# b0nes164/GPUSorting

Hardware: NVIDIA H100
Metric: OneSweep sort throughput, 2^30 uint32 keys per GPU, keys-only, uniform-random (higher is better)
Workload: dtype u32

## Files before the change

### gpusorting_b200/csrc/osb_kernels.cu

```cuda
#include <type_traits>

#include "osb_kernels.cuh"
#include "osb_common.cuh"

namespace osb {

template <typename... Ts> struct TypeList {};

template <typename... Ts, typename F>
static cudaError_t for_each_type(TypeList<Ts...>, F&& f)
{
    cudaError_t e = cudaSuccess;
    (void)(((e = f(Ts{})) == cudaSuccess) && ...);
    return e;
}

template <typename... Ts, typename M, typename F>
static cudaError_t find_type(TypeList<Ts...>, M&& match, F&& f)
{
    cudaError_t e = cudaErrorInvalidValue;
    (void)((match(Ts{}) && ((e = f(Ts{})), true)) || ...);
    return e;
}

template <typename... Keys, typename F>
static cudaError_t with_key_type(TypeList<Keys...> keys, int key_bytes, F&& f)
{
    return find_type(keys, [&](auto k) { return key_bytes == static_cast<int>(sizeof(k)); }, f);
}

template <typename F>
static cudaError_t with_rank_mode(int rank_mode, F&& f)
{
    return rank_mode == kRankBallot ? f(std::integral_constant<int, kRankBallot>{}) : f(std::integral_constant<int, kRankAtomic>{});
}

static unsigned capped_grid(uint64_t work, uint64_t per_cta, uint64_t cap)
{
    uint64_t want = (work + per_cta - 1) / per_cta;
    if (want < 1) want = 1;
    return static_cast<unsigned>(want < cap ? want : cap);
}

constexpr uint64_t kAllResident = ~0ull;
template <auto Kern, int THREADS, size_t SMEM, typename... Args>
static cudaError_t launch_resident(uint64_t max_ctas, int sm_count, cudaStream_t stream, Args... args)
{
    static const int per_sm = [] {
        int b = 0;
        return cudaOccupancyMaxActiveBlocksPerMultiprocessor(&b, Kern, THREADS, SMEM) == cudaSuccess ? b : 0;
    }();
    if (per_sm <= 0) return cudaErrorLaunchOutOfResources;
    const uint64_t ctas = static_cast<uint64_t>(per_sm) * sm_count;
    Kern<<<static_cast<unsigned>(max_ctas < ctas ? max_ctas : ctas), THREADS, SMEM, stream>>>(args...);
    return cudaGetLastError();
}

template <typename K>
static cudaError_t set_smem(K* kernel, size_t bytes)
{
    return cudaFuncSetAttribute(kernel, cudaFuncAttributeMaxDynamicSharedMemorySize, static_cast<int>(bytes));
}

template <typename Shape>
// ... 48 lines not shown
        v.x = enc2(v.x); v.y = enc2(v.y); v.z = enc2(v.z); v.w = enc2(v.w);
    } else {
        unsigned long long k0 = (static_cast<unsigned long long>(v.y) << 32) | v.x, k1 = (static_cast<unsigned long long>(v.w) << 32) | v.z;
        k0 = codec_encode<unsigned long long>(k0, c.a, c.b, c.d); k1 = codec_encode<unsigned long long>(k1, c.a, c.b, c.d);
        v.x = static_cast<uint32_t>(k0); v.y = static_cast<uint32_t>(k0 >> 32); v.z = static_cast<uint32_t>(k1); v.w = static_cast<uint32_t>(k1 >> 32);
    }
    return v;
}

template <typename KeyT, bool MASKED = false>
__device__ __forceinline__ void hist_count_vec(uint32_t* s_col, const uint4& v, int places = 0, uint32_t last_mask = 255u)
{
    hist_count_word<KeyT, MASKED>(s_col, v.x, 0, places, last_mask);
    hist_count_word<KeyT, MASKED>(s_col, v.y, 1, places, last_mask);
    hist_count_word<KeyT, MASKED>(s_col, v.z, 2, places, last_mask);
    hist_count_word<KeyT, MASKED>(s_col, v.w, 3, places, last_mask);
}

template <typename KeyT, bool MASKED = false>
__global__ void __launch_bounds__(kHistThreads, 1)
global_histogram_kernel(const KeyT* __restrict__ keys, uint64_t n, unsigned long long* __restrict__ ghist, KeyCodec codec,
                        int places = 0, uint32_t last_mask = 255u, const SortPlan* gate = nullptr)
{
    if (gate != nullptr && (gate->skip_mask & kPlanFusedKept)) return;
    constexpr int PLACES = sizeof(KeyT);
    constexpr int VEC = 16 / sizeof(KeyT);
    constexpr int COLS = HistGeom<KeyT>::COLS;
    constexpr int BINS = PLACES * kRadix;
    extern __shared__ __align__(16) uint32_t s_hist[];
    for (int i = threadIdx.x; i < BINS * COLS; i += kHistThreads) s_hist[i] = 0;
    __syncthreads();
    uint32_t* s_col = s_hist + (threadIdx.x & (COLS - 1));

    const uint64_t nvec = n / VEC;
    const uint4* __restrict__ vp = reinterpret_cast<const uint4*>(keys);
    const uint64_t stride = static_cast<uint64_t>(gridDim.x) * kHistThreads;
    uint64_t i = static_cast<uint64_t>(blockIdx.x) * kHistThreads + threadIdx.x;
    const bool enc = codec.flags & kCodecEncodeOnLoad;
    for (; i + 3 * stride < nvec; i += 4 * stride) {
        uint4 a = __ldcs(vp + i);
        uint4 b = __ldcs(vp + i + stride);
        uint4 c = __ldcs(vp + i + 2 * stride);
        uint4 d = __ldcs(vp + i + 3 * stride);
        if (enc) { a = hist_encode_vec<KeyT>(a, codec); b = hist_encode_vec<KeyT>(b, codec); c = hist_encode_vec<KeyT>(c, codec); d = hist_encode_vec<KeyT>(d, codec); }
        hist_count_vec<KeyT, MASKED>(s_col, a, places, last_mask);
        hist_count_vec<KeyT, MASKED>(s_col, b, places, last_mask);
// ... 18 lines not shown
            }
        }
    }
    __syncthreads();
    for (int bin = threadIdx.x; bin < BINS; bin += kHistThreads) {
        uint32_t sum = 0;
#pragma unroll 8
        for (int c = 0; c < COLS; ++c) sum += s_hist[bin * COLS + ((c + threadIdx.x) & (COLS - 1))];
        if (sum) atomicAdd(&ghist[bin], static_cast<unsigned long long>(sum));
    }
}

template <typename KeyT> constexpr size_t hist_smem_bytes() { return sizeof(KeyT) * kRadix * HistGeom<KeyT>::COLS * sizeof(uint32_t); }

using HistKeys = TypeList<uint16_t, uint32_t, uint64_t>;
using HistBitsKeys = TypeList<uint32_t, uint64_t>;

template <typename KeyT, bool MASKED>
static cudaError_t launch_histogram_vec(const void* keys, uint64_t n, unsigned long long* ghist, int sm_count, cudaStream_t stream,
                                        const KeyCodec& codec, int places = 0, uint32_t last_mask = 255u,
                                        const SortPlan* gate = nullptr)
{
    const unsigned grid = capped_grid(n / (16 / sizeof(KeyT)), kHistThreads, sm_count);
    global_histogram_kernel<KeyT, MASKED><<<grid, kHistThreads, hist_smem_bytes<KeyT>(), stream>>>(
        static_cast<const KeyT*>(keys), n, ghist, codec, places, last_mask, gate);
    return cudaGetLastError();
}

cudaError_t launch_global_histogram(const void* keys, uint64_t n, int key_bytes, unsigned long long* ghist,
                                    int sm_count, cudaStream_t stream, const KeyCodec* codec_in, const SortPlan* gate)
{
    const KeyCodec codec = codec_in ? *codec_in : KeyCodec();
    return with_key_type(HistKeys{}, key_bytes, [&](auto k) {
        return launch_histogram_vec<decltype(k), false>(keys, n, ghist, sm_count, stream, codec, 0, 255u, gate);
    });
}

__global__ void __launch_bounds__(512)
fused_fallback_zero_kernel(const SortPlan* __restrict__ plan, const uint32_t* __restrict__ ticket, uint32_t ctas, uint64_t tiles,
                           uint4* __restrict__ agg16, uint4* __restrict__ desc)
{
    if (plan->skip_mask & kPlanFusedKept) return;
    uint64_t reached = static_cast<uint64_t>(ctas) + *ticket;
    if (reached > tiles) reached = tiles;
    const uint64_t agg_vecs = (reached + 7) / 8 * 8 * kRadix * sizeof(uint16_t) / 16;
    const uint64_t desc_vecs = reached * kRadix * sizeof(uint64_t) / 16;
    const uint64_t stride = static_cast<uint64_t>(gridDim.x) * blockDim.x;
    for (uint64_t i = static_cast<uint64_t>(blockIdx.x) * blockDim.x + threadIdx.x; i < agg_vecs + desc_vecs; i += stride)
        (i < agg_vecs ? agg16[i] : desc[i - agg_vecs]) = make_uint4(0, 0, 0, 0);
}

cudaError_t launch_fused_fallback_zero(const SortPlan* plan, const uint32_t* ticket, uint32_t ctas, uint64_t tiles, uint16_t* agg16,
                                       uint64_t* desc, int sm_count, cudaStream_t stream)
{
    fused_fallback_zero_kernel<<<static_cast<unsigned>(sm_count) * 4, 512, 0, stream>>>(plan, ticket, ctas, tiles,
                                                                                         reinterpret_cast<uint4*>(agg16),
                                                                                         reinterpret_cast<uint4*>(desc));
    return cudaGetLastError();
}

template <typename KeyT>
__global__ void __launch_bounds__(kHistThreads, 1)
digit_histogram_kernel(const KeyT* __restrict__ keys, uint64_t n, uint32_t shift, unsigned long long* __restrict__ hist256)
{
    __shared__ uint32_t s_hist[kRadix * 32];
    for (int i = threadIdx.x; i < kRadix * 32; i += kHistThreads) s_hist[i] = 0;
    __syncthreads();
    uint32_t* s_col = s_hist + (threadIdx.x & 31);
    const uint64_t stride = static_cast<uint64_t>(gridDim.x) * kHistThreads;
    uint64_t i = static_cast<uint64_t>(blockIdx.x) * kHistThreads + threadIdx.x;
    for (; i + 3 * stride < n; i += 4 * stride) {
        const KeyT a = __ldcs(keys + i), b = __ldcs(keys + i + stride), c = __ldcs(keys + i + 2 * stride),
                   d = __ldcs(keys + i + 3 * stride);
        atomicAdd(&s_col[digit_of(a, shift) * 32], 1u);
        atomicAdd(&s_col[digit_of(b, shift) * 32], 1u);
        atomicAdd(&s_col[digit_of(c, shift) * 32], 1u);
        atomicAdd(&s_col[digit_of(d, shift) * 32], 1u);
    }
    for (; i < n; i += stride) atomicAdd(&s_col[digit_of(__ldcs(keys + i), shift) * 32], 1u);
    __syncthreads();
    for (int bin = threadIdx.x; bin < kRadix; bin += kHistThreads) {
// ... 3 lines not shown
        if (sum) atomicAdd(&hist256[bin], static_cast<unsigned long long>(sum));
    }
}

cudaError_t launch_digit_histogram(const void* keys, uint64_t n, int key_bytes, uint32_t shift,
                                   unsigned long long* hist256, int sm_count, cudaStream_t stream)
{
    const unsigned grid = capped_grid(n, kHistThreads * 4, static_cast<uint64_t>(sm_count) * 2);
    return with_key_type(TypeList<uint32_t, uint64_t>{}, key_bytes, [&](auto k) {
        using KeyT = decltype(k);
        digit_histogram_kernel<KeyT><<<grid, kHistThreads, 0, stream>>>(static_cast<const KeyT*>(keys), n, shift, hist256);
        return cudaGetLastError();
    });
}

enum ScanMode : int { kScanClassic = 0, kScanFused = 1, kScanFallback = 2 };

__global__ void __launch_bounds__(kRadix)
scan_kernel(const unsigned long long* __restrict__ ghist, unsigned long long* __restrict__ gbase, int places,
            SortPlan* plan, unsigned long long n, int allow_skip, int allow_hot, int mode, const uint32_t* fused_abort,
            unsigned long long region)
{
    __shared__ unsigned long long s_warp[kRadix / 32];
    if (mode == kScanFallback && (plan->skip_mask & kPlanFusedKept)) return;
    const int d = threadIdx.x, lane = d & 31, warp = d >> 5;
    uint32_t skip_mask = 0;
    const int overfull = mode == kScanFused ? __syncthreads_or(ghist[d] > region || *fused_abort != 0) : 0;
    for (int p = 0; p < places; ++p) {
        const unsigned long long c = ghist[p * kRadix + d];
        unsigned long long incl = c;
#pragma unroll
        for (int o = 1; o < 32; o <<= 1) {
            const unsigned long long t = __shfl_up_sync(0xffffffffu, incl, o);
            if (lane >= o) incl += t;
        }
        if (lane == 31) s_warp[warp] = incl;
        const int single_bin = __syncthreads_or(plan != nullptr && allow_skip && c == n);
        const int hot_bin = __syncthreads_or(plan != nullptr && allow_hot && n >= (1ull << 22) && c * 8ull >= n);
        unsigned long long pre = 0;
        for (int w = 0; w < warp; ++w) pre += s_warp[w];
        gbase[p * kRadix + d] = pre + incl - c;
        if (single_bin) skip_mask |= 1u << p;
        else if (hot_bin) skip_mask |= 1u << (kPlanHotShift + p);
        __syncthreads();
    }
    if (plan != nullptr && d == 0) {
        SortPlan pl;
        pl.skip_mask = skip_mask;
        const uint32_t run = ~skip_mask & ((places >= 32 ? 0u : (1u << places)) - 1u);
        pl.executed = __popc(run);
        pl.first_exec = run ? static_cast<uint32_t>(__ffs(run) - 1) : 0xffffffffu;
        pl.last_exec = run ? static_cast<uint32_t>(31 - __clz(run)) : 0xffffffffu;
        if (mode == kScanFused && !overfull && (run & 1u) && !((skip_mask >> kPlanHotShift) & 1u) && (run & ~1u))
            pl.skip_mask |= kPlanFusedKept;
        *plan = pl;
    }
}

cudaError_t launch_scan(const unsigned long long* ghist, unsigned long long* gbase, int places, cudaStream_t stream,
                        SortPlan* plan, uint64_t n, bool allow_skip, bool allow_hot)
{
    scan_kernel<<<1, kRadix, 0, stream>>>(ghist, gbase, places, plan, n, allow_skip ? 1 : 0, allow_hot ? 1 : 0, kScanClassic,
                                          nullptr, 0ull);
    return cudaGetLastError();
}

cudaError_t launch_scan_fused(const unsigned long long* ghist, unsigned long long* gbase, int places, cudaStream_t stream,
                              SortPlan* plan, uint64_t n, bool allow_skip, bool allow_hot, bool fallback, const uint32_t* fused_abort,
                              uint64_t region)
{
    scan_kernel<<<1, kRadix, 0, stream>>>(ghist, gbase, places, plan, n, allow_skip ? 1 : 0, allow_hot ? 1 : 0,
                                          fallback ? kScanFallback : kScanFused, fused_abort, region);
    return cudaGetLastError();
}

template <typename KeyT>
__global__ void __launch_bounds__(kHistThreads, 1)
global_histogram_bits_kernel(const KeyT* __restrict__ keys, uint64_t n, unsigned long long* __restrict__ ghist, KeyCodec codec,
                             uint32_t begin_bit, int places, uint32_t last_mask)
{
    constexpr int COLS = HistGeom<KeyT>::COLS;
    extern __shared__ __align__(16) uint32_t s_hist[];
    const int bins = places * kRadix;
    for (int i = threadIdx.x; i < bins * COLS; i += kHistThreads) s_hist[i] = 0;
    __syncthreads();
    uint32_t* s_col = s_hist + (threadIdx.x & (COLS - 1));
    const bool enc = codec.flags & kCodecEncodeOnLoad;
    const KeyT ca = static_cast<KeyT>(codec.a), cb = static_cast<KeyT>(codec.b), cd = static_cast<KeyT>(codec.d);
    const uint64_t stride = static_cast<uint64_t>(gridDim.x) * kHistThreads;
    for (uint64_t i = static_cast<uint64_t>(blockIdx.x) * kHistThreads + threadIdx.x; i < n; i += stride) {
        KeyT k = __ldcs(keys + i);
        if (enc) k = codec_encode<KeyT>(k, ca, cb, cd);
        for (int p = 0; p < places; ++p) {
            const uint32_t dg = digit_of(k, begin_bit + 8u * p, p == places - 1 ? last_mask : 255u);
            atomicAdd(&s_col[(p * kRadix + dg) * COLS], 1u);
        }
    }
    __syncthreads();
    for (int bin = threadIdx.x; bin < bins; bin += kHistThreads) {
        uint32_t sum = 0;
#pragma unroll 8
        for (int c = 0; c < COLS; ++c) sum += s_hist[bin * COLS + ((c + threadIdx.x) & (COLS - 1))];
        if (sum) atomicAdd(&ghist[bin], static_cast<unsigned long long>(sum));
    }
}

cudaError_t launch_global_histogram_bits(const void* keys, uint64_t n, int key_bytes, unsigned long long* ghist, int sm_count,
                                         cudaStream_t stream, const KeyCodec* codec_in, uint32_t begin_bit, int places,
                                         uint32_t last_bits)
{
    const KeyCodec codec = codec_in ? *codec_in : KeyCodec();
    const uint32_t last_mask = (1u << last_bits) - 1u;
    return with_key_type(HistBitsKeys{}, key_bytes, [&](auto k) {
        using KeyT = decltype(k);
        if (begin_bit == 0) return launch_histogram_vec<KeyT, true>(keys, n, ghist, sm_count, stream, codec, places, last_mask);
        global_histogram_bits_kernel<KeyT><<<capped_grid(n, kHistThreads * 4, sm_count), kHistThreads, hist_smem_bytes<KeyT>(), stream>>>(
            static_cast<const KeyT*>(keys), n, ghist, codec, begin_bit, places, last_mask);
        return cudaGetLastError();
    });
}

template <typename W>
__global__ void __launch_bounds__(512)
copy_back_kernel(const SortPlan* __restrict__ plan, const W* __restrict__ src, W* __restrict__ dst, uint64_t words,
                 const unsigned char* __restrict__ src_tail, unsigned char* __restrict__ dst_tail, uint32_t tail_bytes)
{
    if (!(plan->executed & 1u)) return;
    const uint64_t stride = static_cast<uint64_t>(gridDim.x) * blockDim.x;
    for (uint64_t i = static_cast<uint64_t>(blockIdx.x) * blockDim.x + threadIdx.x; i < words; i += stride) __stcs(dst + i, __ldcs(src + i));
    if (blockIdx.x == 0 && threadIdx.x < tail_bytes) dst_tail[threadIdx.x] = src_tail[threadIdx.x];
}

cudaError_t launch_copy_back(const SortPlan* plan, const void* alt_keys, void* keys, const uint32_t* alt_vals, uint32_t* vals,
                             uint64_t n, int key_bytes, int sm_count, cudaStream_t stream)
{
    auto launch = [&](auto word, const void* s, void* d, uint64_t bytes) {
        using W = decltype(word);
        const uint64_t words = bytes / sizeof(W);
        copy_back_kernel<W><<<capped_grid(words, 512, static_cast<uint64_t>(sm_count) * 4), 512, 0, stream>>>(plan, static_cast<const W*>(s), static_cast<W*>(d), words,
                                                      static_cast<const unsigned char*>(s) + words * sizeof(W),
                                                      static_cast<unsigned char*>(d) + words * sizeof(W),
                                                      static_cast<uint32_t>(bytes - words * sizeof(W)));
    };
    auto one = [&](const void* s, void* d, uint64_t bytes) {
        if (((reinterpret_cast<uintptr_t>(s) | reinterpret_cast<uintptr_t>(d)) & 15u) == 0) launch(uint4{}, s, d, bytes);
        else launch(uint32_t{}, s, d, bytes);
    };
    one(alt_keys, keys, n * key_bytes);
    if (vals) one(alt_vals, vals, n * sizeof(uint32_t));
    return cudaGetLastError();
}

template <typename KeyT>
__global__ void __launch_bounds__(512)
argsort_copy_back_kernel(const SortPlan* __restrict__ plan, const KeyT* __restrict__ keys_in, const KeyT* __restrict__ alt_keys,
                         KeyT* __restrict__ keys, const uint32_t* __restrict__ alt_idx, uint32_t* __restrict__ idx, uint64_t n)
{
    using KV = typename std::conditional<sizeof(KeyT) == 2, uint2, uint4>::type;
    constexpr int KV_PER_STEP = 4 * sizeof(KeyT) / sizeof(KV);
    static_assert(KV_PER_STEP * sizeof(KV) == 4 * sizeof(KeyT), "four keys per step");
    const uint32_t ex = plan->executed;
    if (ex != 0 && !(ex & 1u)) return;
    const KeyT* src = ex ? alt_keys : keys_in;
    const uint64_t vecs = n / 4, stride = static_cast<uint64_t>(gridDim.x) * blockDim.x;
    for (uint64_t i = static_cast<uint64_t>(blockIdx.x) * blockDim.x + threadIdx.x; i < vecs; i += stride) {
#pragma unroll
        for (int v = 0; v < KV_PER_STEP; ++v)
            __stcs(reinterpret_cast<KV*>(keys) + i * KV_PER_STEP + v, __ldcs(reinterpret_cast<const KV*>(src) + i * KV_PER_STEP + v));
        const uint32_t b = static_cast<uint32_t>(i * 4);
        __stcs(reinterpret_cast<uint4*>(idx) + i, ex ? __ldcs(reinterpret_cast<const uint4*>(alt_idx) + i) : make_uint4(b, b + 1, b + 2, b + 3));
    }
    if (blockIdx.x == 0 && threadIdx.x < (n & 3u)) {
        const uint64_t j = vecs * 4 + threadIdx.x;
        keys[j] = src[j];
        idx[j] = ex ? alt_idx[j] : static_cast<uint32_t>(j);
    }
}

cudaError_t launch_argsort_copy_back(const SortPlan* plan, const void* keys_in, const void* alt_keys, void* keys,
                                     const uint32_t* alt_idx, uint32_t* idx, uint64_t n, int key_bytes, int sm_count,
                                     cudaStream_t stream)
{
    const unsigned grid = capped_grid(n / 4, 512, static_cast<uint64_t>(sm_count) * 4);
    return with_key_type(TypeList<uint16_t, uint32_t, uint64_t>{}, key_bytes, [&](auto k) {
        using KeyT = decltype(k);
        argsort_copy_back_kernel<KeyT><<<grid, 512, 0, stream>>>(plan, static_cast<const KeyT*>(keys_in), static_cast<const KeyT*>(alt_keys),
                                                                 static_cast<KeyT*>(keys), alt_idx, idx, n);
        return cudaGetLastError();
    });
}


__device__ __forceinline__ uint32_t warp_match_digit(uint32_t d)
{
    uint32_t m = 0xffffffffu;
#pragma unroll
    for (int b = 0; b < kRadixLog; ++b) {
        const bool p = (d >> b) & 1u;
        const uint32_t bal = __ballot_sync(0xffffffffu, p);
        m &= p ? bal : ~bal;
    }
    return m;
}

template <int RANK_MODE>
__device__ __forceinline__ uint32_t warp_rank_and_count(uint32_t* wh, uint32_t d, uint32_t lt_mask)
{
    if constexpr (RANK_MODE == kRankAtomic) {
        (void)lt_mask;
        return atomicAdd(&wh[d], 1u);
    } else {
// ... 258 lines not shown
    for (uint32_t i = 0; i < tile_keys; ++i) {
        KeyT k = p[i];
        if (encode) k = codec_encode<KeyT>(k, ca, cb, cd);
        c += digit_of(k, shift, mask) == d;
    }
    st_relaxed_gpu_u16(dst, kAggReady | c);
    return c;
}

__device__ __forceinline__ uint64_t agg_index(uint64_t tile, uint32_t d) { return ((tile >> 3) * kRadix + d) * 8 + (tile & 7); }

__device__ __forceinline__ uint4 ld_relaxed_gpu_v4(const void* p)
{
    uint4 v;
    asm volatile("ld.relaxed.gpu.global.v4.u32 {%0, %1, %2, %3}, [%4];" : "=r"(v.x), "=r"(v.y), "=r"(v.z), "=r"(v.w) : "l"(p) : "memory");
    return v;
}
__device__ __forceinline__ uint32_t agg_elem(const uint4& v, int t)
{
    const uint32_t w = t < 2 ? v.x : t < 4 ? v.y : t < 6 ? v.z : v.w;
    return (t & 1) ? (w >> 16) : (w & 0xffffu);
}

template <int NBLK, typename KeyT, typename Hook = NoStallHook>
__device__ __forceinline__ unsigned long long
lookback_wide(uint16_t* agg16, const uint64_t* incl64, uint32_t tile, uint32_t d, uint32_t epoch, uint32_t spin_cap,
              const TileRereduce<KeyT>& rr, Hook hook = Hook())
{
    unsigned long long sum = 0;
    int64_t cur = static_cast<int64_t>(tile) - 1;
    uint32_t polls = 0;
    while (true) {
        if (cur < 0) return sum;
#if OSB_PHASE_PROBE
        if (d == 0) atomicAdd(&g_phase[9], 1ull);
#endif
        const int64_t b0 = cur >> 3;
        uint4 v[NBLK];
        uint64_t c[NBLK];
#pragma unroll
        for (int k = 0; k < NBLK; ++k) {
            const int64_t b = b0 - k;
            v[k] = b >= 0 ? ld_relaxed_gpu_v4(agg16 + (static_cast<uint64_t>(b) * kRadix + d) * 8)
                          : make_uint4(0x80008000u, 0x80008000u, 0x80008000u, 0x80008000u);
            c[k] = b > 0 ? ld_relaxed_gpu_u64(incl64 + (static_cast<uint64_t>(b) * 8 - 1) * kRadix + d) : 0ull;
        }
// ... 1 lines not shown
        int64_t next = (b0 - NBLK + 1) * 8 - 1;
        bool stalled = false;
        const int hi0 = static_cast<int>(cur & 7);
#pragma unroll
        for (int k = 0; k < NBLK; ++k) {
            const int64_t b = b0 - k;
            if (b < 0) return run;
#pragma unroll
            for (int t = 7; t >= 0; --t) {
                if (k == 0 && t > hi0) continue;
                const uint32_t a = agg_elem(v[k], t);
                if (!(a & kAggReady)) { next = b * 8 + t; stalled = true; break; }
                run += a & 0x7fffu;
            }
            if (stalled) break;
            if (b == 0) return run;
            if (desc_epoch(c[k]) == epoch && (c[k] & kFlagMask) == kFlagInclusive) return run + desc_value(c[k]);
        }
        sum = run;
        if (stalled) {
            if (hook(-1) == kHookAbort) return sum;
            polls = next == cur ? polls + 1 : 1;
            if (polls > spin_cap) {
                const uint64_t w = ld_relaxed_gpu_u64(incl64 + next * kRadix + d);
                if (desc_epoch(w) == epoch && (w & kFlagMask) == kFlagInclusive) return sum + desc_value(w);
                const long long h = hook(next);
                if (h >= 0)
                    sum += static_cast<unsigned long long>(h);
                else
                    sum += rereduce_tile<KeyT>(rr.in + static_cast<uint64_t>(next) * rr.tile_keys, rr.tile_keys, rr.shift, rr.mask,
                                               rr.encode ? 1u : 0u, rr.ca, rr.cb, rr.cd, agg16 + agg_index(next, d), d);
                --next;
                polls = 0;
            } else {
#if OSB_PHASE_PROBE
                if (d == 0) atomicAdd(&g_phase[10], 1ull);
#endif
                __nanosleep(40);
            }
        } else {
            polls = 0;
        }
        cur = next;
    }
}


constexpr uint32_t kNoHotDigit = 0xffffffffu;
// ... 87 lines not shown
                  (sizeof(KeyT) == 8 && sizeof(S::sorted) == sizeof(KeyT) * T && sizeof(S::sorted_val) == sizeof(uint32_t) * T),
                  "kv layout");
    uint2* const kv = reinterpret_cast<uint2*>(sm.sorted);
    auto put_slot = [&](uint32_t slot, KeyT k, uint32_t v) {
        if constexpr (KV_WORD) kv[slot] = make_uint2(static_cast<uint32_t>(k), v);
        else { sm.sorted[slot] = k; sm.sorted_val[slot] = v; }
    };
    auto get_slot = [&](uint32_t x, KeyT& k, uint32_t& v) {
        if constexpr (KV_WORD) { const uint2 e = kv[x]; k = static_cast<KeyT>(e.x); v = e.y; }
        else { k = sm.sorted[x]; v = sm.sorted_val[x]; }
    };

    const int tid = threadIdx.x, lane = tid & 31, warp = tid >> 5;
    const uint32_t lt = lanemask_lt();
    uint32_t* wh = sm.hist + warp * kRadix;
    const uint32_t shift = pp.shift, epoch = pp.epoch;
    const uint32_t dmask = (1u << pp.dbits) - 1u;
#if OSB_PHASE_PROBE
    long long t_prev = clock64();
#endif

    uint32_t my_bits = (codec.flags & (kCodecEncodeOnLoad | kCodecDecodeOnStore)) << 1;
    bool my_skip = false, my_hot = false;
    if (pp.plan != nullptr) {
        const uint4 raw = __ldg(reinterpret_cast<const uint4*>(pp.plan));
        SortPlan pl; pl.skip_mask = raw.x; pl.executed = raw.y; pl.first_exec = raw.z; pl.last_exec = raw.w;
        my_skip = (pl.skip_mask >> pp.place) & 1u;
        my_hot = (pl.skip_mask >> (kPlanHotShift + pp.place)) & 1u;
        my_bits = plan_src_is_alt(pl, pp.place) ? 1u : 0u;
        if (codec.flags & kCodecFromPlan)
            my_bits |= (pp.place == pl.first_exec ? kCodecEncodeOnLoad << 1 : 0u) | (pp.place == pl.last_exec ? kCodecDecodeOnStore << 1 : 0u);
        if constexpr (INDICES) my_bits |= pp.place == pl.first_exec ? kPlanBitsFirstIndices : 0u;
        if constexpr (S::kFusable) my_bits |= plan_reads_gapped(pl, pp.place) ? kPlanBitsGapped : 0u;
        if (pp.place == 0 && (pl.skip_mask & kPlanFusedKept)) my_skip = true;
    }
    if (my_skip) return;
    if (HOT != my_hot) return;
    const uint32_t num_tiles = static_cast<uint32_t>((n + T - 1) / T);

    using KeyReg = typename std::conditional<sizeof(KeyT) == 2 && !PAIRS, uint32_t, KeyT>::type;
    KeyReg key[K];
    uint32_t val[PAIRS ? K : 1];
    const uint32_t warp_off = warp * (32 * K) + lane;
    auto region_of = [&](uint64_t p) {
        uint32_t r = 0;
#pragma unroll 1
// ... 126 lines not shown

    auto chained_scan = [&]() {
        if (tid < kRadix) {
            TileRereduce<KeyT> rr;
            rr.in = (INDICES && (sm.plan_bits & kPlanBitsFirstIndices)) ? static_cast<const KeyT*>(pp.keys_in)
                    : (sm.plan_bits & 1u) ? buf1 : buf0;
            rr.tile_keys = T; rr.shift = shift; rr.mask = dmask;
            rr.encode = (sm.plan_bits >> 1) & kCodecEncodeOnLoad;
            rr.ca = static_cast<KeyT>(codec.a); rr.cb = static_cast<KeyT>(codec.b); rr.cd = static_cast<KeyT>(codec.d);
            auto hook = [&](long long t) -> long long {
                if (t < 0) {
                    if constexpr (FUSED) return *reinterpret_cast<const volatile uint32_t*>(pp.fused_abort) ? kHookAbort : kHookDefault;
                    return kHookDefault;
                }
                if (S::kFusable && (sm.plan_bits & kPlanBitsGapped))
                    return rereduce_tile_gapped<KeyT>(buf1, static_cast<uint64_t>(t) * T, T, shift, dmask, pp.dense_base0, pp.region,
                                                      agg16 + agg_index(t, tid), tid);
                return kHookDefault;
            };
            const unsigned long long prior = lookback_wide<LOOK / 8, KeyT>(agg16, incl64, tile, tid, epoch, pp.spin_cap, rr, hook);
            const bool swap = sm.plan_bits & 1u;
            KeyT* out = swap ? buf0 : buf1;
            uint32_t* out_val = swap ? val0 : val1;
            st_relaxed_gpu_u64(incl64 + static_cast<uint64_t>(tile) * kRadix + tid,
                               desc_pack(epoch, kFlagInclusive, prior + tile_count));
            if constexpr (FUSED) {
                const uint32_t live_d = tile_count - ((tid == kRadix - 1 && !full) ? (T - valid) : 0u);
                fused_count += live_d;
                if (prior + live_d > pp.region || live_d > T / 16) {
                    *reinterpret_cast<volatile uint32_t*>(pp.fused_abort) = 1u;
                    sm.fused_stop = 1u;
                } else if (*reinterpret_cast<const volatile uint32_t*>(pp.fused_abort)) {
                    sm.fused_stop = 1u;
                }
            }
            const unsigned long long first = (FUSED ? tid * pp.region : gbase[tid]) + prior - tile_excl;
            sm.keyptr[tid] = reinterpret_cast<unsigned long long>(out) + first * sizeof(KeyT);
            if constexpr (PAIRS) sm.valptr[tid] = reinterpret_cast<unsigned long long>(out_val) + first * sizeof(uint32_t);
            if (tid < 32) {
                const uint32_t pad_digit = digit_of(static_cast<KeyT>(~static_cast<KeyT>(0)), shift, dmask);
                const uint32_t live = tile_count - ((tid == pad_digit && !full) ? (T - valid) : 0u);
                sm.run[tid] = tile_excl | (live << 16);
            }
        }
    };

    constexpr bool kRecompute = RANK_MODE == kRankAtomic && !HOT;
    const uint32_t rshift = kRecompute ? opaque_copy(&sm.digit_shift) : shift;
// ... 9 lines not shown
            const uint32_t b = __ballot_sync(0xffffffffu, is_hot);
            uint32_t slot = hot_run + __popc(b & lt);
            if (!is_hot) slot = warp_rank_and_count<RANK_MODE>(wh, d, lt);
            hot_run += __popc(b);
            if constexpr (PAIRS) put_slot(slot, key[i], val[i]);
            else sm.sorted[slot] = key[i];
        }
    } else {
#pragma unroll
        for (int i = 0; i < K; ++i) {
            const uint32_t slot = warp_rank_and_count<RANK_MODE>(wh, digit_of(key[i], rshift, rmask), lt);
            if constexpr (PAIRS) put_slot(slot, key[i], val[i]);
            else sm.sorted[slot] = key[i];
        }
    }
    __syncwarp();
    {
        uint4* r4 = reinterpret_cast<uint4*>(wh);
#pragma unroll
        for (int i = lane; i < kRadix / 4; i += 32) r4[i] = make_uint4(0, 0, 0, 0);
    }

    const uint32_t next = sm.next_tile;
    if constexpr (kPersistent) { if (!HOT || warp >= kRadix / 32) load_tile(next); }
    OSB_PHASE(4);
    if constexpr (FUSED) {
        if (warp < kRadix / 32) {
            named_bar_arrive(1, THREADS);
        } else {
            named_bar_sync(1, THREADS);
            const uint4* s4 = reinterpret_cast<const uint4*>(sm.sorted);
#pragma unroll 1
            for (uint32_t j = tid - kRadix; j < T / 4; j += THREADS - kRadix) {
                const uint4 v = s4[j];
                const uint32_t w[4] = {v.x, v.y, v.z, v.w};
#pragma unroll
                for (int q = 0; q < 4; ++q) {
                    if (full || 4 * j + q < valid) {
                        atomicAdd(&sm.fhist[(w[q] >> 8) & 255u], 1u);
                        atomicAdd(&sm.fhist[kRadix + ((w[q] >> 16) & 255u)], 1u);
                        atomicAdd(&sm.fhist[2 * kRadix + (w[q] >> 24)], 1u);
                    }
                }
            }
        }
    }
// ... 194 lines not shown
            st_relaxed_gpu_u16(agg16 + agg_index(tile, tid), kAggReady | tile_count);
    }
    tile_excl = block_excl_scan_256<THREADS>(tile_count, sm.wtot);
    if (tid < kRadix) {
        uint32_t run = tile_excl;
#pragma unroll
        for (int w = 0; w < WARPS; ++w) { const uint32_t c = sm.hist[w * kRadix + tid]; sm.hist[w * kRadix + tid] = run; run += c; }
    }
    __syncthreads();

    uint32_t slots[K / 2];
#pragma unroll
    for (int i = 0; i < K; ++i) {
        const uint32_t slot = warp_rank_and_count<RANK_MODE>(wh, digit_of(key[i], shift, dmask), lt);
        sm.sorted[slot] = key[i];
        if (i & 1) slots[i / 2] |= slot << 16; else slots[i / 2] = slot;
    }
    if (tid < kRadix) {
        TileRereduce<KeyT> rr;
        rr.in = (sm.plan_bits & 1u) ? buf1 : buf0; rr.tile_keys = T; rr.shift = shift; rr.mask = dmask;
        rr.encode = (sm.plan_bits >> 1) & kCodecEncodeOnLoad;
        rr.ca = static_cast<KeyT>(codec.a); rr.cb = static_cast<KeyT>(codec.b); rr.cd = static_cast<KeyT>(codec.d);
        const unsigned long long prior = lookback_wide<LOOK / 8, KeyT>(agg16, incl64, tile, tid, epoch, pp.spin_cap, rr);
        st_relaxed_gpu_u64(incl64 + static_cast<uint64_t>(tile) * kRadix + tid, desc_pack(epoch, kFlagInclusive, prior + tile_count));
        const bool swap = sm.plan_bits & 1u;
        const unsigned long long first = gbase[tid] + prior - tile_excl;
        sm.keyptr[tid] = reinterpret_cast<unsigned long long>(swap ? buf0 : buf1) + first * sizeof(KeyT);
        sm.valptr[tid] = reinterpret_cast<unsigned long long>(swap ? val0 : val1) + first * sizeof(uint32_t);
    }
    __syncthreads();

    asm volatile("" ::: "memory");
    {
        const uint32_t* __restrict__ in_val = (sm.plan_bits & 1u) ? val1 : val0;
        if (full) {
#pragma unroll
            for (int i = 0; i < K; ++i) key[i] = ld_stream(in_val + tile_base + warp_off + i * 32);
        } else {
#pragma unroll
            for (int i = 0; i < K; ++i) {
                const uint32_t idx = warp_off + i * 32;
                key[i] = idx < valid ? in_val[tile_base + idx] : 0u;
            }
        }
    }

    {
// ... 133 lines not shown

        uint32_t tile_count = 0, tile_excl = 0;
        if (tid < kRadix) {
#pragma unroll
            for (int w = 0; w < WARPS; ++w) tile_count += sm.hist[w * kRadix + tid];
            st_relaxed_gpu_u16(agg16 + agg_index(tile, tid), kAggReady | tile_count);
        }
        tile_excl = block_excl_scan_256<THREADS>(tile_count, sm.wtot);
        if (tid < kRadix) {
            uint32_t run = tile_excl;
#pragma unroll
            for (int w = 0; w < WARPS; ++w) { const uint32_t c = sm.hist[w * kRadix + tid]; sm.hist[w * kRadix + tid] = run; run += c; }
        }
        __syncthreads();

#pragma unroll
        for (int i = 0; i < K; ++i) s_keys[warp_rank_and_count<RANK_MODE>(wh, digit_of(key[i], shift), lt)] = key[i];

        if (tid < kRadix) {
            TileRereduce<KeyT> rr;
            rr.in = in; rr.tile_keys = T; rr.shift = shift; rr.mask = kRadix - 1; rr.encode = false;
            rr.ca = rr.cb = rr.cd = 0;
            const unsigned long long prior = lookback_wide<LOOK / 8, KeyT>(agg16, incl64, tile, tid, epoch, 1u << 20, rr);
            st_relaxed_gpu_u64(incl64 + static_cast<uint64_t>(tile) * kRadix + tid,
                               desc_pack(epoch, kFlagInclusive, prior + tile_count));
            sm.keyptr[tid] = reinterpret_cast<unsigned long long>(out) + (gbase[tid] + prior - tile_excl) * sizeof(KeyT);
        }
        __syncthreads();

        if (full) {
#pragma unroll
            for (int j = 0; j < K; ++j) {
                const uint32_t idx = j * THREADS + tid;
                const KeyT k = s_keys[idx];
                st_stream(reinterpret_cast<KeyT*>(sm.keyptr[digit_of(k, shift)]) + idx, k);
            }
        } else {
#pragma unroll 4
            for (int j = 0; j < K; ++j) {
                const uint32_t idx = j * THREADS + tid;
                if (idx < valid) {
                    const KeyT k = s_keys[idx];
                    st_stream(reinterpret_cast<KeyT*>(sm.keyptr[digit_of(k, shift)]) + idx, k);
                }
            }
        }
        zero_hist();
        __syncthreads();
// ... 108 lines not shown
    static constexpr bool has_hot = true;
    template <int RANK_MODE, bool HOT = false>
    static auto kernel() { return digit_binning_wide_kernel<KeyT, PAIRS, G::K, G::WARPS, RANK_MODE, G::LOOK, G::MINB, HOT, INDICES>; }
    template <int RANK_MODE>
    static cudaError_t launch(const PassArgs& a)
    {
        const uint64_t tiles = (a.n + T - 1) / T;
        const PassParams pp = a.params();
        auto grid_for = [&](auto kernel, int& per_sm, bool persistent) -> unsigned {
            if (!persistent) return static_cast<unsigned>(tiles);
            if (per_sm == 0) {
                int b = 0;
                if (cudaOccupancyMaxActiveBlocksPerMultiprocessor(&b, kernel, S::THREADS, smem) != cudaSuccess || b < 1) b = 1;
                per_sm = b;
            }
            uint64_t cap = static_cast<uint64_t>(a.cfg.sm_count) * per_sm;
            if (a.cfg.debug_max_ctas && a.cfg.debug_max_ctas < cap) cap = a.cfg.debug_max_ctas;
            return static_cast<unsigned>(tiles < cap ? tiles : cap);
        };
        KeyT* buf0 = static_cast<KeyT*>(const_cast<void*>(a.in));
        uint32_t* val0 = const_cast<uint32_t*>(a.in_val);
        const auto kern = kernel<RANK_MODE>();
        static int plain_per_sm = 0;
        kern<<<grid_for(kern, plain_per_sm, sizeof(KeyT) <= 4 && !PAIRS), S::THREADS, smem, a.stream>>>(
            buf0, static_cast<KeyT*>(a.out), val0, a.out_val, a.n, a.gbase, a.agg16, a.desc, a.ticket, pp, a.cfg.codec);
        if (a.cfg.plan != nullptr && a.cfg.hot_passes) {
            const auto hot = kernel<RANK_MODE, true>();
            static int hot_per_sm = 0;
            hot<<<grid_for(hot, hot_per_sm, true), S::THREADS, smem, a.stream>>>(
                buf0, static_cast<KeyT*>(a.out), val0, a.out_val, a.n, a.gbase, a.agg16, a.desc, a.ticket, pp, a.cfg.codec);
        }
        return cudaGetLastError();
    }
};

constexpr int kPairsK = 32, kPairsWarps = 16;

struct Pairs16KShape : PassShape<uint32_t, true> {
    static constexpr bool enabled = OSB_PAIRS16K != 0;
    using S = PairsSmem<kPairsWarps, kPairsK>;
    static constexpr uint32_t T = S::T;
    static constexpr size_t smem = sizeof(S);
    template <int RANK_MODE, bool HOT = false>
    static auto kernel() { return digit_binning_pairs_kernel<kPairsK, kPairsWarps, RANK_MODE, OSB_PAIRS_LOOK>; }
    template <int RANK_MODE>
    static cudaError_t launch(const PassArgs& a)
    {
        const auto kern = kernel<RANK_MODE>();
        kern<<<static_cast<unsigned>((a.n + T - 1) / T), S::THREADS, smem, a.stream>>>(
            static_cast<uint32_t*>(const_cast<void*>(a.in)), static_cast<uint32_t*>(a.out), const_cast<uint32_t*>(a.in_val), a.out_val,
            a.n, a.gbase, a.agg16, a.desc, a.ticket, a.params(), a.cfg.codec);
        return cudaGetLastError();
    }
};

// ... 85 lines not shown
        static int per_sm = 0;
        if (per_sm == 0) {
            int b = 0;
            if (cudaOccupancyMaxActiveBlocksPerMultiprocessor(&b, kern, FusedShape::S::THREADS, FusedShape::smem) != cudaSuccess || b < 1) b = 1;
            per_sm = b;
        }
        const uint64_t tiles = (n + FusedShape::T - 1) / FusedShape::T;
        uint64_t cap = static_cast<uint64_t>(cfg.sm_count) * per_sm;
        if (cfg.debug_max_ctas && cfg.debug_max_ctas < cap) cap = cfg.debug_max_ctas;
        PassParams pp;
        pp.shift = 0;
        pp.dbits = 8;
        pp.epoch = epoch;
        pp.place = 0;
        pp.spin_cap = cfg.spin_cap;
        pp.stall_every = cfg.debug_stall_every;
        pp.plan = nullptr;
        pp.region = region;
        pp.fused_abort = abort_word;
        pp.fused_hist = ghist;
        KeyCodec codec = cfg.codec;
        codec.flags &= kCodecEncodeOnLoad;
        *ctas = static_cast<uint32_t>(tiles < cap ? tiles : cap);
        kern<<<*ctas, FusedShape::S::THREADS, FusedShape::smem, stream>>>(
            const_cast<uint32_t*>(keys), alt, nullptr, nullptr, n, nullptr, agg16, desc, ticket, pp, codec);
        return cudaGetLastError();
    });
}

cudaError_t launch_digit_binning(const void* in, void* out, const uint32_t* in_val, uint32_t* out_val, uint64_t n,
                                 int key_bytes, uint32_t shift, const unsigned long long* gbase_place, uint64_t* desc,
                                 uint16_t* agg16, uint32_t* ticket, uint32_t epoch, const BinningConfig& cfg,
                                 cudaStream_t stream)
{
    const bool pairs = in_val != nullptr;
    if (cfg.variant != kVariantWide && (cfg.codec.flags || cfg.plan != nullptr || cfg.debug_stall_every || cfg.argsort_in))
        return cudaErrorNotSupported;
    if (cfg.digit_bits < 1 || cfg.digit_bits > 8) return cudaErrorInvalidValue;
    if (cfg.variant != kVariantWide && cfg.digit_bits != 8 && shift + cfg.digit_bits != static_cast<uint32_t>(key_bytes) * 8u)
        return cudaErrorNotSupported;
    const bool indices = cfg.argsort_in != nullptr;
    if (indices && (!pairs || cfg.plan == nullptr)) return cudaErrorInvalidValue;
    const PassArgs a{in, out, in_val, out_val, n, shift, gbase_place, desc, agg16, ticket, epoch, cfg, stream};
    return with_rank_mode(cfg.rank_mode, [&](auto r) {
        return with_pass_shape(key_bytes, pairs, indices, cfg.variant,
                               [&](auto s) { return decltype(s)::template launch<decltype(r)::value>(a); });
    });
}

// ... 2656 lines not shown
```

Before: 68.15.

## Chain sort kernels with programmatic dependent launch and thin inclusive descriptor stores

Launches the histogram, scan, binning, fallback and copy-back kernels with programmatic stream serialization. Each kernel calls griddepcontrol wait/launch_dependents, so the next kernel's launch and prologue can overlap the tail of the previous one. Separately, the lookback now writes and reads inclusive descriptors only for every eighth tile, which cuts global stores but can make lookback fall back to aggregates more often. The early-release placement in the binning kernel relies on correct wait ordering in consumers.

New measurement: 68.81, median of 6. No clear change (+1.0%).

```diff
diff --git a/gpusorting_b200/csrc/osb_kernels.cu b/gpusorting_b200/csrc/osb_kernels.cu
--- a/gpusorting_b200/csrc/osb_kernels.cu
+++ b/gpusorting_b200/csrc/osb_kernels.cu
@@ -1,4 +1,5 @@
 #include <type_traits>
+#include <utility>
 
 #include "osb_kernels.cuh"
 #include "osb_common.cuh"
@@ -40,6 +41,26 @@
     uint64_t want = (work + per_cta - 1) / per_cta;
     if (want < 1) want = 1;
     return static_cast<unsigned>(want < cap ? want : cap);
+}
+
+__device__ __forceinline__ void chain_wait() { asm volatile("griddepcontrol.wait;" ::: "memory"); }
+__device__ __forceinline__ void chain_release() { asm volatile("griddepcontrol.launch_dependents;" ::: "memory"); }
+
+template <typename... P, typename... A>
+static cudaError_t launch_chained(void (*kernel)(P...), unsigned grid, unsigned threads, size_t smem, cudaStream_t stream,
+                                  A&&... args)
+{
+    cudaLaunchAttribute attr[1];
+    attr[0].id = cudaLaunchAttributeProgrammaticStreamSerialization;
+    attr[0].val.programmaticStreamSerializationAllowed = 1;
+    cudaLaunchConfig_t cfg = {};
+    cfg.gridDim = dim3(grid);
+    cfg.blockDim = dim3(threads);
+    cfg.dynamicSmemBytes = smem;
+    cfg.stream = stream;
+    cfg.attrs = attr;
+    cfg.numAttrs = 1;
+    return cudaLaunchKernelEx(&cfg, kernel, std::forward<A>(args)...);
 }
 
 constexpr uint64_t kAllResident = ~0ull;
@@ -134,6 +155,8 @@
 global_histogram_kernel(const KeyT* __restrict__ keys, uint64_t n, unsigned long long* __restrict__ ghist, KeyCodec codec,
                         int places = 0, uint32_t last_mask = 255u, const SortPlan* gate = nullptr)
 {
+    chain_release();
+    chain_wait();
     if (gate != nullptr && (gate->skip_mask & kPlanFusedKept)) return;
     constexpr int PLACES = sizeof(KeyT);
     constexpr int VEC = 16 / sizeof(KeyT);
@@ -198,9 +221,8 @@
                                         const SortPlan* gate = nullptr)
 {
     const unsigned grid = capped_grid(n / (16 / sizeof(KeyT)), kHistThreads, sm_count);
-    global_histogram_kernel<KeyT, MASKED><<<grid, kHistThreads, hist_smem_bytes<KeyT>(), stream>>>(
-        static_cast<const KeyT*>(keys), n, ghist, codec, places, last_mask, gate);
-    return cudaGetLastError();
+    return launch_chained(global_histogram_kernel<KeyT, MASKED>, grid, kHistThreads, hist_smem_bytes<KeyT>(), stream,
+                          static_cast<const KeyT*>(keys), n, ghist, codec, places, last_mask, gate);
 }
 
 cudaError_t launch_global_histogram(const void* keys, uint64_t n, int key_bytes, unsigned long long* ghist,
@@ -216,6 +238,8 @@
 fused_fallback_zero_kernel(const SortPlan* __restrict__ plan, const uint32_t* __restrict__ ticket, uint32_t ctas, uint64_t tiles,
                            uint4* __restrict__ agg16, uint4* __restrict__ desc)
 {
+    chain_release();
+    chain_wait();
     if (plan->skip_mask & kPlanFusedKept) return;
     uint64_t reached = static_cast<uint64_t>(ctas) + *ticket;
     if (reached > tiles) reached = tiles;
@@ -229,10 +253,8 @@
 cudaError_t launch_fused_fallback_zero(const SortPlan* plan, const uint32_t* ticket, uint32_t ctas, uint64_t tiles, uint16_t* agg16,
                                        uint64_t* desc, int sm_count, cudaStream_t stream)
 {
-    fused_fallback_zero_kernel<<<static_cast<unsigned>(sm_count) * 4, 512, 0, stream>>>(plan, ticket, ctas, tiles,
-                                                                                         reinterpret_cast<uint4*>(agg16),
-                                                                                         reinterpret_cast<uint4*>(desc));
-    return cudaGetLastError();
+    return launch_chained(fused_fallback_zero_kernel, static_cast<unsigned>(sm_count) * 4, 512, 0, stream, plan, ticket, ctas, tiles,
+                          reinterpret_cast<uint4*>(agg16), reinterpret_cast<uint4*>(desc));
 }
 
 template <typename KeyT>
@@ -282,6 +304,8 @@
             unsigned long long region)
 {
     __shared__ unsigned long long s_warp[kRadix / 32];
+    chain_release();
+    chain_wait();
     if (mode == kScanFallback && (plan->skip_mask & kPlanFusedKept)) return;
     const int d = threadIdx.x, lane = d & 31, warp = d >> 5;
     uint32_t skip_mask = 0;
@@ -320,18 +344,18 @@
 cudaError_t launch_scan(const unsigned long long* ghist, unsigned long long* gbase, int places, cudaStream_t stream,
                         SortPlan* plan, uint64_t n, bool allow_skip, bool allow_hot)
 {
-    scan_kernel<<<1, kRadix, 0, stream>>>(ghist, gbase, places, plan, n, allow_skip ? 1 : 0, allow_hot ? 1 : 0, kScanClassic,
-                                          nullptr, 0ull);
-    return cudaGetLastError();
+    return launch_chained(scan_kernel, 1, kRadix, 0, stream, ghist, gbase, places, plan, static_cast<unsigned long long>(n),
+                          allow_skip ? 1 : 0, allow_hot ? 1 : 0, static_cast<int>(kScanClassic), static_cast<const uint32_t*>(nullptr),
+                          0ull);
 }
 
 cudaError_t launch_scan_fused(const unsigned long long* ghist, unsigned long long* gbase, int places, cudaStream_t stream,
                               SortPlan* plan, uint64_t n, bool allow_skip, bool allow_hot, bool fallback, const uint32_t* fused_abort,
                               uint64_t region)
 {
-    scan_kernel<<<1, kRadix, 0, stream>>>(ghist, gbase, places, plan, n, allow_skip ? 1 : 0, allow_hot ? 1 : 0,
-                                          fallback ? kScanFallback : kScanFused, fused_abort, region);
-    return cudaGetLastError();
+    return launch_chained(scan_kernel, 1, kRadix, 0, stream, ghist, gbase, places, plan, static_cast<unsigned long long>(n),
+                          allow_skip ? 1 : 0, allow_hot ? 1 : 0, static_cast<int>(fallback ? kScanFallback : kScanFused), fused_abort,
+                          static_cast<unsigned long long>(region));
 }
 
 template <typename KeyT>
@@ -341,6 +365,8 @@
 {
     constexpr int COLS = HistGeom<KeyT>::COLS;
     extern __shared__ __align__(16) uint32_t s_hist[];
+    chain_release();
+    chain_wait();
     const int bins = places * kRadix;
     for (int i = threadIdx.x; i < bins * COLS; i += kHistThreads) s_hist[i] = 0;
     __syncthreads();
@@ -374,9 +400,9 @@
     return with_key_type(HistBitsKeys{}, key_bytes, [&](auto k) {
         using KeyT = decltype(k);
         if (begin_bit == 0) return launch_histogram_vec<KeyT, true>(keys, n, ghist, sm_count, stream, codec, places, last_mask);
-        global_histogram_bits_kernel<KeyT><<<capped_grid(n, kHistThreads * 4, sm_count), kHistThreads, hist_smem_bytes<KeyT>(), stream>>>(
-            static_cast<const KeyT*>(keys), n, ghist, codec, begin_bit, places, last_mask);
-        return cudaGetLastError();
+        return launch_chained(global_histogram_bits_kernel<KeyT>, capped_grid(n, kHistThreads * 4, sm_count), kHistThreads,
+                              hist_smem_bytes<KeyT>(), stream, static_cast<const KeyT*>(keys), n, ghist, codec, begin_bit, places,
+                              last_mask);
     });
 }
 
@@ -385,6 +411,7 @@
 copy_back_kernel(const SortPlan* __restrict__ plan, const W* __restrict__ src, W* __restrict__ dst, uint64_t words,
                  const unsigned char* __restrict__ src_tail, unsigned char* __restrict__ dst_tail, uint32_t tail_bytes)
 {
+    chain_wait();
     if (!(plan->executed & 1u)) return;
     const uint64_t stride = static_cast<uint64_t>(gridDim.x) * blockDim.x;
     for (uint64_t i = static_cast<uint64_t>(blockIdx.x) * blockDim.x + threadIdx.x; i < words; i += stride) __stcs(dst + i, __ldcs(src + i));
@@ -397,18 +424,17 @@
     auto launch = [&](auto word, const void* s, void* d, uint64_t bytes) {
         using W = decltype(word);
         const uint64_t words = bytes / sizeof(W);
-        copy_back_kernel<W><<<capped_grid(words, 512, static_cast<uint64_t>(sm_count) * 4), 512, 0, stream>>>(plan, static_cast<const W*>(s), static_cast<W*>(d), words,
-                                                      static_cast<const unsigned char*>(s) + words * sizeof(W),
-                                                      static_cast<unsigned char*>(d) + words * sizeof(W),
-                                                      static_cast<uint32_t>(bytes - words * sizeof(W)));
+        return launch_chained(copy_back_kernel<W>, capped_grid(words, 512, static_cast<uint64_t>(sm_count) * 4), 512, 0, stream, plan,
+                              static_cast<const W*>(s), static_cast<W*>(d), words, static_cast<const unsigned char*>(s) + words * sizeof(W),
+                              static_cast<unsigned char*>(d) + words * sizeof(W), static_cast<uint32_t>(bytes - words * sizeof(W)));
     };
     auto one = [&](const void* s, void* d, uint64_t bytes) {
-        if (((reinterpret_cast<uintptr_t>(s) | reinterpret_cast<uintptr_t>(d)) & 15u) == 0) launch(uint4{}, s, d, bytes);
-        else launch(uint32_t{}, s, d, bytes);
+        if (((reinterpret_cast<uintptr_t>(s) | reinterpret_cast<uintptr_t>(d)) & 15u) == 0) return launch(uint4{}, s, d, bytes);
+        return launch(uint32_t{}, s, d, bytes);
     };
-    one(alt_keys, keys, n * key_bytes);
-    if (vals) one(alt_vals, vals, n * sizeof(uint32_t));
-    return cudaGetLastError();
+    const cudaError_t e = one(alt_keys, keys, n * key_bytes);
+    if (e != cudaSuccess || !vals) return e;
+    return one(alt_vals, vals, n * sizeof(uint32_t));
 }
 
 template <typename KeyT>
@@ -419,6 +445,7 @@
     using KV = typename std::conditional<sizeof(KeyT) == 2, uint2, uint4>::type;
     constexpr int KV_PER_STEP = 4 * sizeof(KeyT) / sizeof(KV);
     static_assert(KV_PER_STEP * sizeof(KV) == 4 * sizeof(KeyT), "four keys per step");
+    chain_wait();
     const uint32_t ex = plan->executed;
     if (ex != 0 && !(ex & 1u)) return;
     const KeyT* src = ex ? alt_keys : keys_in;
@@ -444,9 +471,8 @@
     const unsigned grid = capped_grid(n / 4, 512, static_cast<uint64_t>(sm_count) * 4);
     return with_key_type(TypeList<uint16_t, uint32_t, uint64_t>{}, key_bytes, [&](auto k) {
         using KeyT = decltype(k);
-        argsort_copy_back_kernel<KeyT><<<grid, 512, 0, stream>>>(plan, static_cast<const KeyT*>(keys_in), static_cast<const KeyT*>(alt_keys),
-                                                                 static_cast<KeyT*>(keys), alt_idx, idx, n);
-        return cudaGetLastError();
+        return launch_chained(argsort_copy_back_kernel<KeyT>, grid, 512, 0, stream, plan, static_cast<const KeyT*>(keys_in),
+                              static_cast<const KeyT*>(alt_keys), static_cast<KeyT*>(keys), alt_idx, idx, n);
     });
 }
 
@@ -751,6 +777,8 @@
     return (t & 1) ? (w >> 16) : (w & 0xffffu);
 }
 
+__device__ __forceinline__ bool incl_published(uint64_t tile) { return (tile & 7) == 7; }
+
 template <int NBLK, typename KeyT, typename Hook = NoStallHook>
 __device__ __forceinline__ unsigned long long
 lookback_wide(uint16_t* agg16, const uint64_t* incl64, uint32_t tile, uint32_t d, uint32_t epoch, uint32_t spin_cap,
@@ -798,8 +826,10 @@
             if (hook(-1) == kHookAbort) return sum;
             polls = next == cur ? polls + 1 : 1;
             if (polls > spin_cap) {
-                const uint64_t w = ld_relaxed_gpu_u64(incl64 + next * kRadix + d);
-                if (desc_epoch(w) == epoch && (w & kFlagMask) == kFlagInclusive) return sum + desc_value(w);
+                if (incl_published(static_cast<uint64_t>(next))) {
+                    const uint64_t w = ld_relaxed_gpu_u64(incl64 + next * kRadix + d);
+                    if (desc_epoch(w) == epoch && (w & kFlagMask) == kFlagInclusive) return sum + desc_value(w);
+                }
                 const long long h = hook(next);
                 if (h >= 0)
                     sum += static_cast<unsigned long long>(h);
@@ -933,6 +963,7 @@
 
     uint32_t my_bits = (codec.flags & (kCodecEncodeOnLoad | kCodecDecodeOnStore)) << 1;
     bool my_skip = false, my_hot = false;
+    chain_wait();
     if (pp.plan != nullptr) {
         const uint4 raw = __ldg(reinterpret_cast<const uint4*>(pp.plan));
         SortPlan pl; pl.skip_mask = raw.x; pl.executed = raw.y; pl.first_exec = raw.z; pl.last_exec = raw.w;
@@ -1105,8 +1136,9 @@
             const bool swap = sm.plan_bits & 1u;
             KeyT* out = swap ? buf0 : buf1;
             uint32_t* out_val = swap ? val0 : val1;
-            st_relaxed_gpu_u64(incl64 + static_cast<uint64_t>(tile) * kRadix + tid,
-                               desc_pack(epoch, kFlagInclusive, prior + tile_count));
+            if (incl_published(tile))
+                st_relaxed_gpu_u64(incl64 + static_cast<uint64_t>(tile) * kRadix + tid,
+                                   desc_pack(epoch, kFlagInclusive, prior + tile_count));
             if constexpr (FUSED) {
                 const uint32_t live_d = tile_count - ((tid == kRadix - 1 && !full) ? (T - valid) : 0u);
                 fused_count += live_d;
@@ -1162,6 +1194,7 @@
     }
 
     const uint32_t next = sm.next_tile;
+    if (next >= num_tiles) chain_release();
     if constexpr (kPersistent) { if (!HOT || warp >= kRadix / 32) load_tile(next); }
     OSB_PHASE(4);
     if constexpr (FUSED) {
@@ -1402,7 +1435,8 @@
         rr.encode = (sm.plan_bits >> 1) & kCodecEncodeOnLoad;
         rr.ca = static_cast<KeyT>(codec.a); rr.cb = static_cast<KeyT>(codec.b); rr.cd = static_cast<KeyT>(codec.d);
         const unsigned long long prior = lookback_wide<LOOK / 8, KeyT>(agg16, incl64, tile, tid, epoch, pp.spin_cap, rr);
-        st_relaxed_gpu_u64(incl64 + static_cast<uint64_t>(tile) * kRadix + tid, desc_pack(epoch, kFlagInclusive, prior + tile_count));
+        if (incl_published(tile))
+            st_relaxed_gpu_u64(incl64 + static_cast<uint64_t>(tile) * kRadix + tid, desc_pack(epoch, kFlagInclusive, prior + tile_count));
         const bool swap = sm.plan_bits & 1u;
         const unsigned long long first = gbase[tid] + prior - tile_excl;
         sm.keyptr[tid] = reinterpret_cast<unsigned long long>(swap ? buf0 : buf1) + first * sizeof(KeyT);
@@ -1582,8 +1616,9 @@
             rr.in = in; rr.tile_keys = T; rr.shift = shift; rr.mask = kRadix - 1; rr.encode = false;
             rr.ca = rr.cb = rr.cd = 0;
             const unsigned long long prior = lookback_wide<LOOK / 8, KeyT>(agg16, incl64, tile, tid, epoch, 1u << 20, rr);
-            st_relaxed_gpu_u64(incl64 + static_cast<uint64_t>(tile) * kRadix + tid,
-                               desc_pack(epoch, kFlagInclusive, prior + tile_count));
+            if (incl_published(tile))
+                st_relaxed_gpu_u64(incl64 + static_cast<uint64_t>(tile) * kRadix + tid,
+                                   desc_pack(epoch, kFlagInclusive, prior + tile_count));
             sm.keyptr[tid] = reinterpret_cast<unsigned long long>(out) + (gbase[tid] + prior - tile_excl) * sizeof(KeyT);
         }
         __syncthreads();
@@ -1738,15 +1773,16 @@
         uint32_t* val0 = const_cast<uint32_t*>(a.in_val);
         const auto kern = kernel<RANK_MODE>();
         static int plain_per_sm = 0;
-        kern<<<grid_for(kern, plain_per_sm, sizeof(KeyT) <= 4 && !PAIRS), S::THREADS, smem, a.stream>>>(
-            buf0, static_cast<KeyT*>(a.out), val0, a.out_val, a.n, a.gbase, a.agg16, a.desc, a.ticket, pp, a.cfg.codec);
-        if (a.cfg.plan != nullptr && a.cfg.hot_passes) {
+        cudaError_t e = launch_chained(kern, grid_for(kern, plain_per_sm, sizeof(KeyT) <= 4 && !PAIRS), S::THREADS, smem, a.stream,
+                                       buf0, static_cast<KeyT*>(a.out), val0, a.out_val, a.n, a.gbase, a.agg16, a.desc, a.ticket, pp,
+                                       a.cfg.codec);
+        if (e == cudaSuccess && a.cfg.plan != nullptr && a.cfg.hot_passes) {
             const auto hot = kernel<RANK_MODE, true>();
             static int hot_per_sm = 0;
-            hot<<<grid_for(hot, hot_per_sm, true), S::THREADS, smem, a.stream>>>(
-                buf0, static_cast<KeyT*>(a.out), val0, a.out_val, a.n, a.gbase, a.agg16, a.desc, a.ticket, pp, a.cfg.codec);
-        }
-        return cudaGetLastError();
+            e = launch_chained(hot, grid_for(hot, hot_per_sm, true), S::THREADS, smem, a.stream, buf0, static_cast<KeyT*>(a.out), val0,
+                               a.out_val, a.n, a.gbase, a.agg16, a.desc, a.ticket, pp, a.cfg.codec);
+        }
+        return e;
     }
 };
 
@@ -1878,9 +1914,9 @@
         KeyCodec codec = cfg.codec;
         codec.flags &= kCodecEncodeOnLoad;
         *ctas = static_cast<uint32_t>(tiles < cap ? tiles : cap);
-        kern<<<*ctas, FusedShape::S::THREADS, FusedShape::smem, stream>>>(
-            const_cast<uint32_t*>(keys), alt, nullptr, nullptr, n, nullptr, agg16, desc, ticket, pp, codec);
-        return cudaGetLastError();
+        return launch_chained(kern, *ctas, FusedShape::S::THREADS, FusedShape::smem, stream, const_cast<uint32_t*>(keys), alt,
+                              static_cast<uint32_t*>(nullptr), static_cast<uint32_t*>(nullptr), n,
+                              static_cast<const unsigned long long*>(nullptr), agg16, desc, ticket, pp, codec);
     });
 }
 
```
